# srisarya/nanopore-barcoding-ORC

Measured on AMD Instinct MI355X. Metric: Mreads/s two-round SP5×SP27 demux; % HBM roofline; 1/2/4/8 GPU, higher is better.
Workload: dtype u64

## Files before the change

### nanopore-barcoding-orc_amd/csrc/dmx_api.cpp

```cpp
#include <hip/hip_runtime.h>

#include <algorithm>
#include <atomic>
#include <cstdlib>
#include <cstdio>
#include <cstring>
#include <map>
#include <mutex>
#include <thread>
#include <tuple>
#include <utility>
#include <vector>

#include "dmx_internal.h"
#include "pack.h"

using namespace dmx;

#define CK(call)                                                                        \
    do {                                                                                \
        hipError_t e_ = (call);                                                         \
        if (e_ != hipSuccess) {                                                         \
            c->err = std::string(#call) + ": " + hipGetErrorString(e_);                 \
            return DMX_E_HIP;                                                           \
// ... 38 lines not shown


size_t counts_size(const Ctx* c) {
    const size_t a1 = c->mode == DMX_MODE_SINGLE ? 0 : (size_t)c->panel[1].n;
    return ((size_t)c->panel[0].n + 1) * (a1 + 1) + 2;
}

int ensure_pipeline(Ctx* c) {
    const size_t n = c->n_reads;
    const bool linked = c->mode == DMX_MODE_LINKED;
    const size_t slots0 = linked ? n * (size_t)std::max(1, c->panel[0].n) : n;
    const size_t items = linked ? slots0 : n;
    const size_t need = std::max(slots0, items) * (linked ? 1 : 2);
    if (!c->d_res || c->res_cap < n) {
        int rc;
        if ((rc = dev_alloc(c, &c->d_res, n))) return rc;
        c->res_cap = n;
    }
    if (c->slot_cap < need || c->cap_reads < n) {
        const size_t s = need;
        int rc;
        for (int r = 0; r < 2; ++r) {
            if ((rc = dev_alloc(c, &c->d_winner[r], s))) return rc;
            if ((rc = dev_alloc(c, &c->d_origin[r], s))) return rc;
            if ((rc = dev_alloc(c, &c->d_lb[r], s))) return rc;
        }
        if ((rc = dev_alloc(c, &c->d_linked, n))) return rc;
        c->slot_cap = s;
        c->cap_reads = n;
    }
    if (c->item_alloc < items) {
        int rc;
        if ((rc = dev_alloc(c, &c->d_items, items))) return rc;
        c->item_alloc = items;
    }
    c->item_cap = items;
    const size_t want_cl = 4 * std::max(slots0, n) + 65536;
    if (c->cl_cap < want_cl) {
        int rc;
        for (int r = 0; r < 2; ++r) {
            if ((rc = dev_alloc(c, &c->d_cl[r], want_cl))) return rc;
            if ((rc = dev_alloc(c, &c->d_outc[r], want_cl))) return rc;
        }
        c->cl_cap = want_cl;
    }
    const size_t want_cand = 4 * std::max(slots0, n) + 65536;
    if (c->cand_cap < want_cand) {
        int rc;
        for (int r = 0; r < 2; ++r)
            for (int l = 0; l < 2; ++l) {
                if ((rc = dev_alloc(c, &c->d_cand[r][l], want_cand))) return rc;
                if ((rc = dev_alloc(c, &c->d_cand_out[r][l], want_cand))) return rc;
            }
        c->cand_cap = want_cand;
    }
    const size_t want_win = 4 * 2 * std::max(slots0, n) + 65536;
    if (c->win_cap < want_win) {
        int rc;
        if ((rc = dev_alloc(c, &c->d_win, want_win))) return rc;
        if ((rc = dev_alloc(c, &c->d_win2, want_win))) return rc;
        if ((rc = dev_alloc(c, &c->d_tasks, 4 * want_win))) return rc;
        if ((rc = dev_alloc(c, &c->d_ftask, want_win))) return rc;
        c->win_cap = want_win;
        c->task_cap = 4 * want_win;
        c->ftask_cap = want_win;
    }
    const size_t want_stage = std::min<size_t>(c->win_cap, 2 * std::max(slots0, n) + 65536);
    if (c->use_stage && c->stage_cap < want_stage) {
        int rc;
        if ((rc = dev_alloc(c, &c->d_stage, want_stage * kStageWords))) return rc;
        c->stage_cap = want_stage;
    }
    const size_t nc = counts_size(c);
    if (c->n_counts != nc) {
        int rc;
// ... 16 lines not shown
                                          : x >= kShTasks ? c->task_cap : c->win_cap) /
                                         kShards);
        uint64_t t = 0;
        for (int s = 0; s < kShards; ++s) {
            const uint32_t v = sh[(size_t)(x * kShards + s) * kShardStride];
            t += std::min(v, scap);
            if (v > scap) o |= cand ? 8 : 4;
        }
        const int slot = x < kShWin2 ? 4 + x : x < kShTasks ? 10 + (x - kShWin2)
                       : x < kShCand ? 12 + (x - kShTasks) : x < kShFtask ? 6 + (x - kShCand)
                       : 14 + (x - kShFtask);
        cnt[slot] = (uint32_t)t;
    }
    if (ovf) *ovf = o;
    return hipSuccess;
}

int grow_cands(Ctx* c) {
    const size_t want = c->cand_cap * 2;
    int rc;
    for (int r = 0; r < 2; ++r)
        for (int l = 0; l < 2; ++l) {
            if ((rc = dev_alloc(c, &c->d_cand[r][l], want))) return rc;
            if ((rc = dev_alloc(c, &c->d_cand_out[r][l], want))) return rc;
        }
    c->cand_cap = want;
    return DMX_OK;
}

int grow_windows(Ctx* c) {
    const size_t want = c->win_cap * 2;
    int rc;
    if ((rc = dev_alloc(c, &c->d_win, want))) return rc;
    if ((rc = dev_alloc(c, &c->d_win2, want))) return rc;
    if ((rc = dev_alloc(c, &c->d_tasks, 4 * want))) return rc;
    if ((rc = dev_alloc(c, &c->d_ftask, want))) return rc;
    c->win_cap = want;
    c->task_cap = 4 * want;
    c->ftask_cap = want;
    return DMX_OK;
}

int grow_clusters(Ctx* c) {
    const size_t want = c->cl_cap * 2;
    int rc;
    for (int r = 0; r < 2; ++r) {
        if ((rc = dev_alloc(c, &c->d_cl[r], want))) return rc;
// ... 98 lines not shown
    hipMalloc((void**)&c->d_shard, kShLists * kShards * kShardStride * sizeof(uint32_t));
    *out = c;
    return DMX_OK;
}

void dmx_close(dmx_ctx* c) {
    if (!c) return;
    hipSetDevice(c->device);
    hipStreamSynchronize(c->stream);
    chop_release(c);
    pd_release(c);
    comm_release(c);
    void* bufs[] = {c->d_seq_alloc, c->d_nmask_alloc,     c->d_offs,     c->d_lens,      c->d_res,
                    c->d_winner[0], c->d_winner[1], c->d_origin[0], c->d_origin[1], c->d_lb[0], c->d_lb[1], c->d_cl[0],
                    c->d_cl[1],     c->d_outc[0],   c->d_outc[1],  c->d_items, c->d_win, c->d_win2, c->d_linked, c->d_tasks, c->d_counters, c->d_shard,
                    c->d_counts,    c->d_panel[0],  c->d_panel[1], c->d_pieces[0], c->d_pieces[1],
                    c->d_ftask, c->d_stage, c->d_pieces_flat, c->d_cells[0], c->d_cells[1], c->d_cells[2],
                    c->d_cells[3]};
    for (void* b : bufs)
        if (b) hipFree(b);
    for (int r = 0; r < 2; ++r)
        for (int l = 0; l < 2; ++l) {
            if (c->d_cand[r][l]) hipFree(c->d_cand[r][l]);
            if (c->d_cand_out[r][l]) hipFree(c->d_cand_out[r][l]);
        }
    void* alt[] = {c->alt.seq_alloc, c->alt.nmask_alloc, c->alt.offs, c->alt.lens, c->alt.res,
                   c->alt.exc, c->d_exc};
    for (void* b : alt)
        if (b) hipFree(b);
    for (auto& e : c->ev)
        if (e) hipEventDestroy(e);
    if (c->cstream) hipStreamDestroy(c->cstream);
    if (c->dstream) hipStreamDestroy(c->dstream);
    hipStreamDestroy(c->stream);
    delete c;
}

const char* dmx_last_error(dmx_ctx* c) {
    if (c) return c->err.c_str();
    thread_local std::string msg;
    msg = dmx::process_error();
    if (msg.empty()) msg = "null context";
    return msg.c_str();
}

int dmx_set_mode(dmx_ctx* c, int mode) {
    if (!c) return DMX_E_INVALID;
// ... 1194 lines not shown
```

### nanopore-barcoding-orc_amd/csrc/dmx_device.h

```cpp
#pragma once
#include <hip/hip_runtime.h>
#include <stdint.h>

namespace dmx {

constexpr int kMaxAdapters = 64;
constexpr int kMaxLen = 64;
constexpr int kRingSmall = 74;
constexpr int kRingLarge = 128;
constexpr int kScanBlock = 256;
constexpr int kResolveBlock = 64;

enum : uint8_t { kFront = 1, kBack = 2 };

struct DevAdapter {
    uint64_t peq[8];
    int8_t acc[72];
    int8_t pacc[72];
    uint8_t m;
    uint8_t k;
    uint8_t where;
    int8_t kk;
    uint8_t pad[4];
};
// ... 154 lines not shown
    uint32_t n, start, len;
    uint8_t strand, o, a, clean;
    uint64_t off;
};
static_assert(sizeof(Cand) == 40 && offsetof(Cand, off) == 32, "Cand layout");

struct Outcome {
    uint64_t key;
    int32_t origin;
    int32_t pad;
};

__host__ __device__ inline uint64_t make_key(int score, int o, int cost, int a, uint64_t t) {
    const int s = score < -128 ? -128 : score;
    return ((uint64_t)(127 - s) << 56) | ((uint64_t)o << 55) | ((uint64_t)cost << 48) |
           ((uint64_t)a << 40) | (t & ((1ull << 40) - 1));
}
__host__ __device__ inline int key_score(uint64_t k) { return 127 - (int)(k >> 56); }
__host__ __device__ inline int key_orient(uint64_t k) { return (int)((k >> 55) & 1); }
__host__ __device__ inline int key_cost(uint64_t k) { return (int)((k >> 48) & 127); }
__host__ __device__ inline int key_adapter(uint64_t k) { return (int)((k >> 40) & 255); }
__host__ __device__ inline uint64_t key_t(uint64_t k) { return k & ((1ull << 40) - 1); }

enum BoundsBuf : uint32_t {
    kBufSeq = 1, kBufMask = 2, kBufSlot = 3, kBufItem = 4, kBufRes = 5, kBufCount = 6,
    kBufRead = 7, kBufLinked = 8, kBufCand = 9, kBufChop = 10, kBufPd = 11,
    kBufPaTrace = 12, kBufPaOps = 13, kBufGaCols = 14, kBufRdCols = 15
};
enum BoundsKernel : int32_t {
    kKerFilter = 1, kKerVerify, kKerScreen, kKerScreen4, kKerWscan, kKerScan, kKerBand0,
    kKerBand1, kKerSelectCand, kKerResolve, kKerSelect, kKerFin0, kKerFin1, kKerFin0L, kKerFin1L,
    kKerFin2L, kKerChop, kKerChopBig, kKerChopStart, kKerSelfTest, kKerPieces, kKerPairdist,
    kKerPairalign, kKerPairalignTb, kKerGroupalign, kKerGroupalignTb, kKerGroupalignMerge,
    kKerRowdist
};
constexpr int kBoundsRec = 24;

struct Bounds {
#ifdef DMX_DEBUG_BOUNDS
    int64_t lo, hi;
    uint64_t slots, items, reads, counts, linked;
    uint32_t* rec;
    int32_t kid;
#endif
};

__device__ __forceinline__ bool bchk(const Bounds& b, int64_t i, int64_t lo, int64_t hi,
                                     uint32_t buf) {
#ifdef DMX_DEBUG_BOUNDS
    if (i >= lo && i < hi) return true;
    atomicOr(b.rec + 3, 32u);
    if (atomicCAS(b.rec + kBoundsRec, 0u, (uint32_t)b.kid + 1u) == 0u) {
        b.rec[kBoundsRec + 1] = buf;
        b.rec[kBoundsRec + 2] = (uint32_t)(uint64_t)i;
// ... 139 lines not shown
```

### nanopore-barcoding-orc_amd/csrc/dmx_internal.h

```cpp
#pragma once
#include <hip/hip_runtime.h>

#include <string>
#include <vector>

#include "../../include/dmx.h"
#include "dmx_device.h"

struct ncclComm;

namespace dmx {

struct ChopState;
struct PdState;
struct PaState;
struct GaState;
struct RdState;

struct PanelReach {
    int pre_raw = 0;
    int pre = 0;
    int post = 0;
    int need_pre = 0;
    int need_post = 0;
// ... 39 lines not shown
    uint32_t* d_seq_alloc = nullptr;
    uint32_t* d_nmask_alloc = nullptr;
    uint64_t* d_offs = nullptr;
    uint32_t* d_lens = nullptr;
    uint32_t* d_exc = nullptr;
    size_t exc_cap = 0;

    struct InSet {
        uint32_t* seq_alloc = nullptr;
        uint32_t* nmask_alloc = nullptr;
        uint64_t* offs = nullptr;
        uint32_t* lens = nullptr;
        dmx_result* res = nullptr;
        uint32_t* exc = nullptr;
        size_t cap_words = 0, cap_reads = 0, res_cap = 0, n_words = 0, exc_cap = 0;
    } alt;
    hipStream_t cstream = nullptr;
    hipStream_t dstream = nullptr;
    bool chunked = false;

    dmx_result* d_res = nullptr;
    unsigned long long* d_winner[2] = {nullptr, nullptr};
    int32_t* d_origin[2] = {nullptr, nullptr};
    int32_t* d_lb[2] = {nullptr, nullptr};
    bool ring_small[2] = {true, true};
    bool band_ok[2] = {true, true};
    bool band_wide[2] = {true, true};
    bool orient_slot[2] = {false, false};
    bool force_ring = false;
    size_t slot_cap = 0;
    Cluster* d_cl[2] = {nullptr, nullptr};
    Outcome* d_outc[2] = {nullptr, nullptr};
    size_t cl_cap = 0;
    Cand* d_cand[2][2] = {{nullptr, nullptr}, {nullptr, nullptr}};
    Outcome* d_cand_out[2][2] = {{nullptr, nullptr}, {nullptr, nullptr}};
    size_t cand_cap = 0;
    Window* d_win = nullptr;
    Window* d_win2 = nullptr;
    size_t win_cap = 0;
    ItemView* d_items = nullptr;
    size_t item_cap = 0;
    size_t item_alloc = 0;
    uint32_t* d_shard = nullptr;
    uint32_t* d_counters = nullptr;
    unsigned long long* d_counts = nullptr;
    unsigned long long* d_linked = nullptr;
    Window* d_tasks = nullptr;
    size_t task_cap = 0;
    uint32_t* d_stage = nullptr;
    size_t stage_cap = 0;
    bool use_stage = false;
    FTask* d_ftask = nullptr;
    size_t ftask_cap = 0;
    DevPieces* d_pieces_flat = nullptr;
    int flat_rounds = 0;
    int flat_want = 0;
    int flat_step = 0;
    size_t flat_lds = 0;
// ... 6 lines not shown
    bool screen_v1 = false;
    size_t n_counts = 0;
    hipEvent_t ev[17] = {};
    bool executed = false;
    ChopState* chop = nullptr;
    PdState* pd = nullptr;
    PaState* pa = nullptr;
    GaState* ga = nullptr;
    RdState* rd = nullptr;

    ncclComm* comm = nullptr;
    int comm_ranks = 0, comm_rank = 0;
    uint64_t comm_group = 0;
    bool counts_reduced = false;
};

void chop_release(Ctx* c);
void pd_release(Ctx* c);
void comm_release(Ctx* c);
int reset_counts(Ctx* c);
void set_process_error(const std::string& msg);
std::string process_error();
void chop_invalidate(Ctx* c);
int launch_round(Ctx* c, int round, hipStream_t st);
int prepare_flat(Ctx* c, hipStream_t st);
int launch_finalize(Ctx* c, int round, hipStream_t st);
int launch_rebase_offsets(uint64_t* offs, uint32_t n, uint64_t g0, hipStream_t st);
int launch_mask_scatter(uint32_t* mask, const uint32_t* d_exc, uint32_t n, uint32_t base,
                        hipStream_t st);

Bounds make_bounds(const Ctx* c, int kid);
inline void set_kid(Bounds& b, int kid) {
#ifdef DMX_DEBUG_BOUNDS
    b.kid = kid;
#else
    (void)b, (void)kid;
#endif
}
hipError_t bounds_reset(Ctx* c, hipStream_t st);
int bounds_check(Ctx* c, const char* where);

PanelReach panel_reach(const HostPanel& hp, const DevPanel& dp);
int bounds_selftest(Ctx* c, uint32_t* host_out);

struct MaskSrc {
    const uint32_t* dense = nullptr;
// ... 13 lines not shown
```

### nanopore-barcoding-orc_amd/csrc/dmx_kernels.hip

```cpp
#include <algorithm>
#include <cstring>
#include <memory>
#include <type_traits>
#include <utility>
#include <vector>

#include "dmx_device.h"
#include "dmx_internal.h"

namespace dmx {

struct RoundArgs {
    Packed pk;
    const uint64_t* offs;
    const uint32_t* lens;
    const DevPanel* panel;
    const ItemView* items;
    const uint32_t* n_items_dev;
    uint32_t n_items;
    int32_t T;
    int32_t per_task_slot;
    int32_t slot_div;
    Cluster* cl;
    Outcome* outc;
    uint32_t* cl_count;
    uint32_t cl_cap;
    uint32_t* flags;
    unsigned long long* winner;
    int32_t* origin;
    int32_t* lb;
    Window* win;
    uint32_t* win_count;
    uint32_t win_cap;
    uint32_t win_scap;
    Window* win2;
    uint32_t* win2_count;
    uint32_t* diag;
    int32_t band;
    Cand* cand[2];
    Outcome* cand_out[2];
    uint32_t* cand_count;
    uint32_t cand_cap;
    uint32_t cand_scap;
    int32_t screen;
    Window* tasks;
    uint32_t* task_count;
    uint32_t task_cap;
    uint32_t task_scap;
    const DevPieces* pieces;
    FTask* ftask;
    uint32_t* ftask_count;
    uint32_t ftask_scap;
    uint32_t* stage;
    uint32_t stage_cap;
    uint32_t n_words;
    uint32_t nsb;
    int32_t round;
    uint32_t* cells[4];
};

#ifndef DMX_MASK_SKIP
#define DMX_MASK_SKIP 1
#endif
// ... 3341 lines not shown
    for (int x = threadIdx.x; x < 72 * A; x += blockDim.x) s_bacc[x] = P->ad[x / 72].acc[x % 72];
    __shared__ uint32_t s_multi;
    if (threadIdx.x == 0) s_multi = 0;
    __syncthreads();
    for (int x = threadIdx.x; x < 64 * A; x += blockDim.x) {
        const int a = x >> 6, i = x & 63;
        const DevAdapter& ad = P->ad[a];
        uint32_t r = 0;
        for (int c = 0; c < 4; ++c) r |= (uint32_t)((ad.peq[c] >> i) & 1ull) << c;
        if (__popc(r) == 1) r |= (uint32_t)(__ffs(r) - 1) << 4;
        else if (i < (int)ad.m) s_multi = 1u;
        s_rm[i * kMaxAdapters + a] = (uint8_t)r;
    }
    if (threadIdx.x == 0) {
        s_nq[0] = 0;
        s_nq[1] = 0;
        s_n = 0;
    }
    __shared__ uint32_t s_spre[kShards + 1];
    ShardMap sm{s_spre, 0u};
    sm.load(R.cand_count + list * kShards * kShardStride, R.cand_scap);
    const uint32_t total = sm.total();
    const Cand* cl = R.cand[list];
    Outcome* outs = R.cand_out[list];
    const uint32_t wave = threadIdx.x >> 6;
    const bool fast = s_multi == 0;

    auto dp_pass = [&](int e, uint32_t cnt) {
        const uint32_t lo = s_nq[e] - cnt;
        if (threadIdx.x < 8) s_hist[threadIdx.x] = 0;
        __syncthreads();
        uint32_t ci = 0, cost = 0, pos = 0;
        const bool have = threadIdx.x < cnt;
        if (have) {
            ci = s_q[e][lo + threadIdx.x];
            cost = s_qc[e][lo + threadIdx.x];
            pos = atomicAdd(&s_hist[cost], 1u);
        }
        __syncthreads();
        if (have) {
            uint32_t before = 0;
            for (uint32_t c = 0; c < cost; ++c) before += s_hist[c];
            s_sorted[before + pos] = ci;
            s_sc[before + pos] = (uint8_t)cost;
        }
        __syncthreads();
        if (threadIdx.x == 0) {
// ... 18 lines not shown
                tv.n = c.n;
                tv.strand = c.strand;
                tv.clean = c.clean != 0;
                tv.start = c.start;
                tv.len = c.len;
                view_off(R.pk, c.off, tv);
                tv.o = c.o;
                tv.a = c.a;
                int c2, origin, score;
#ifdef DMX_BAND_SKIP_DP
                c2 = cst;
                origin = (int)(c.j) - iend;
                score = (int)wc;
                if (false)
#endif
                if (e == 0)
                    band_dp_cost<CMIN == 0 ? 1 : CMIN, CMAX, false>(
                        wc, fast, s_rm + c.a, R.pk, tv, ad.front, iend, j, c2,
                        origin, score);
                else
                    band_dp_cost<CMIN == 0 ? 1 : CMIN, CMAX, true>(
                        wc, fast, s_rm + c.a, R.pk, tv, ad.front, iend, j, c2,
                        origin, score);
                if (c2 != cst) atomicOr(R.flags, 2u);
                const int lr = iend + (origin < 0 ? origin : 0);
                if (slot_in && lr >= 0 && cst <= (int)acc[lr]) {
                    Outcome out;
                    out.key = make_key(score, c.o, cst, c.a, t);
                    out.origin = origin;
                    out.pad = (int32_t)slot;
                    atomicMin(&R.winner[slot], (unsigned long long)out.key);
                    outs[cj] = out;
                }
            }
        }
        __syncthreads();
    };

    for (uint32_t base = blockIdx.x * blockDim.x; base < total; base += gridDim.x * blockDim.x) {
        const uint32_t ti = base + threadIdx.x;
        const uint32_t ci = ti < total ? sm.phys(ti) : 0u;
        Cand c{};
        if (ti < total) c = cl[ci];
        if (ti < total && (cmask == 0 || ((cmask >> c.cost) & 1))) {
            const uint32_t slot = slot_of(R, c.item, c.sub);
            const bool slot_in = DMX_BOUND(R.pk.bd, slots, slot, kBufSlot);
            const int cost = c.cost, iend = c.iend;
            const int j = (int)c.j;
            const uint64_t t = iend == (int)(s_amk[c.a] & 255u) ? (uint64_t)j
                                                               : (uint64_t)c.len + 1 + iend;
            Outcome out;
            out.key = ~0ull;
            out.origin = 0;
            out.pad = 0;
            const int lrmax = min(iend, j + cost);
            const int ub = lrmax - 2 * cost;
            if (slot_in && viable_lb(R.lb[slot], lrmax, c.o, cost) &&
                make_key(ub, c.o, cost, c.a, t) <= R.winner[slot]) {
                if (cost == 0) {
                    const int origin = j - iend;
                    const int score = j >= iend ? iend : j;
                    const int lr = iend + (origin < 0 ? origin : 0);
                    if (lr >= 0 && 0 <= (int)s_bacc[72 * c.a + lr]) {
                        out.key = make_key(score, c.o, 0, c.a, t);
                        out.origin = origin;
                        out.pad = (int32_t)slot;
                        atomicMin(&R.winner[slot], (unsigned long long)out.key);
                    }
                } else {
                    const int dx = j - iend;
                    const int H = CMAX;
                    const int e = (dx - H < 0 || j + H > (int)c.len) ? 1 : 0;
                    const uint32_t q = atomicAdd(&s_nq[e], 1u);
                    s_q[e][q] = ci;
                    s_qc[e][q] = (uint8_t)cost;
                }
            }
            outs[ci] = out;
        }
        __syncthreads();
        for (int e = 0; e < 2; ++e)
            while (s_nq[e] >= 256u) dp_pass(e, 256u);
        __syncthreads();
    }
    for (int e = 0; e < 2; ++e)
        if (s_nq[e]) dp_pass(e, s_nq[e]);
    if (threadIdx.x == 0 && s_n) atomicAdd(R.diag + 1, s_n);
}

__global__ void select_cand_kernel(RoundArgs R) {
    __shared__ uint32_t s_spre[kShards + 1];
    for (int list = 0; list < 2; ++list) {
        ShardMap sm{s_spre, 0u};
        __syncthreads();
        sm.load(R.cand_count + list * kShards * kShardStride, R.cand_scap);
        const uint32_t total = sm.total();
        for (uint32_t ti = blockIdx.x * blockDim.x + threadIdx.x; ti < total;
             ti += gridDim.x * blockDim.x) {
            const uint32_t ci = sm.phys(ti);
            const Outcome o = R.cand_out[list][ci];
            if (o.key == ~0ull) continue;
            const uint32_t slot = (uint32_t)o.pad;
            if (!DMX_BOUND(R.pk.bd, slots, slot, kBufSlot)) continue;
            if (R.winner[slot] == o.key) R.origin[slot] = o.origin;
        }
    }
}

__global__ void select_kernel(RoundArgs R) {
    const uint32_t total = min(*R.cl_count, R.cl_cap);
    for (uint32_t ci = blockIdx.x * blockDim.x + threadIdx.x; ci < total;
         ci += gridDim.x * blockDim.x) {
        const Outcome o = R.outc[ci];
        if (o.key == ~0ull) continue;
        const Cluster c = R.cl[ci];
        const uint32_t slot = slot_of(R, c.item, c.sub);
        if (!DMX_BOUND(R.pk.bd, slots, slot, kBufSlot)) continue;
        if (R.winner[slot] == o.key) R.origin[slot] = o.origin;
    }
}

__device__ __forceinline__ void decode_match(uint64_t key, int origin, uint32_t vlen,
                                             const DevPanel* P, dmx_match& mt, int& a, int& o) {
    a = key_adapter(key);
    o = key_orient(key);
    const uint64_t t = key_t(key);
    int refstop, qstop;
    if (t <= vlen) {
        qstop = (int)t;
        refstop = P->ad[a].m;
    } else {
        refstop = (int)(t - vlen - 1);
        qstop = (int)vlen;
    }
    mt.rstop = qstop;
    mt.astop = (int16_t)refstop;
    if (origin >= 0) {
        mt.astart = 0;
        mt.rstart = origin;
    } else {
        mt.astart = (int16_t)(-origin);
        mt.rstart = 0;
    }
    mt.score = (int16_t)key_score(key);
    mt.errors = (int16_t)key_cost(key);
}

struct FinalArgs {
    const uint32_t* lens;
    const DevPanel* p0;
    const DevPanel* p1;
    const unsigned long long* winner;
    const int32_t* origin;
    dmx_result* res;
    ItemView* items;
    uint32_t* n_items;
    uint32_t n_reads;
    int32_t mode;
    int32_t A0, A1;
    int32_t oslot;
    unsigned long long* counts;
    const unsigned long long* winner0;
    const int32_t* origin0;
    unsigned long long* linked_best;
    Bounds bd;
};

__global__ __launch_bounds__(256) void finalize0_linked_kernel(FinalArgs F) {
    __shared__ uint32_t s_nq, s_qbase;
    if (threadIdx.x == 0) s_nq = 0;
    __syncthreads();
    const uint32_t r = blockIdx.x * blockDim.x + threadIdx.x;
    uint32_t nmine = 0, qi = 0;
    uint32_t n = 0;
    if (r < F.n_reads && DMX_BOUND(F.bd, reads, r, kBufRes) &&
        DMX_BOUND(F.bd, linked, r, kBufLinked) &&
        DMX_BOUND(F.bd, slots, (size_t)r * F.A0 + F.A0 - 1, kBufSlot)) {
        dmx_result out;
        out.bin1 = out.bin2 = -1;
        out.rc1 = out.rc2 = 0;
        out.flags = 0;
        out._pad = 0;
        out.m1 = dmx_match{0, 0, 0, 0, 0, 0};
        out.m2 = out.m1;
        F.res[r] = out;
        F.linked_best[r] = ~0ull;
        n = F.lens[r];
        for (int a = 0; a < F.A0; ++a) nmine += F.winner[(size_t)r * F.A0 + a] != ~0ull;
        if (nmine) qi = atomicAdd(&s_nq, nmine);
    }
    __syncthreads();
    if (threadIdx.x == 0) s_qbase = s_nq ? atomicAdd(F.n_items, s_nq) : 0u;
    __syncthreads();
    if (nmine) {
        uint32_t idx = s_qbase + qi;
        for (int a = 0; a < F.A0; ++a) {
            const uint64_t key = F.winner[(size_t)r * F.A0 + a];
            if (key == ~0ull) continue;
            dmx_match m;
            int aa, o;
            decode_match(key, F.origin[(size_t)r * F.A0 + a], n, F.p0, m, aa, o);
            ItemView v;
            v.read = r;
            v.strand = 0;
            v.pad = 0;
            v.only_adapter = (int16_t)a;
            v.start = (uint32_t)m.rstop;
            v.len = n - (uint32_t)m.rstop;
            if (DMX_BOUND(F.bd, items, idx, kBufItem)) F.items[idx] = v;
            ++idx;
        }
    }
}

__global__ __launch_bounds__(256) void finalize1_linked_kernel(FinalArgs F) {
    const uint32_t i = blockIdx.x * blockDim.x + threadIdx.x;
    if (i >= *F.n_items) return;
    if (!DMX_BOUND(F.bd, items, i, kBufItem) || !DMX_BOUND(F.bd, slots, i, kBufSlot)) return;
    const ItemView v = F.items[i];
    const uint64_t kb = F.winner[i];
    if (kb == ~0ull) return;
    const int a = v.only_adapter;
    if (!DMX_BOUND(F.bd, linked, v.read, kBufLinked)) return;
    const uint64_t kf = F.winner0[(size_t)v.read * F.A0 + a];
// ... 1 lines not shown
    const int err = key_cost(kf) + key_cost(kb);
    const uint64_t ck = ((uint64_t)(511 - sum) << 54) | ((uint64_t)err << 46) |
                        ((uint64_t)a << 38) | (uint64_t)i;
    atomicMin(&F.linked_best[v.read], (unsigned long long)ck);
}

__global__ __launch_bounds__(256) void finalize2_linked_kernel(FinalArgs F) {
    __shared__ unsigned int s_hist[kMaxAdapters + 1];
    for (int x = threadIdx.x; x <= F.A0; x += blockDim.x) s_hist[x] = 0;
    __syncthreads();
    for (uint32_t r = blockIdx.x * blockDim.x + threadIdx.x; r < F.n_reads;
         r += gridDim.x * blockDim.x) {
        const uint64_t ck = DMX_BOUND(F.bd, linked, r, kBufLinked) ? F.linked_best[r] : ~0ull;
        int b = -1;
        if (ck != ~0ull) {
            const uint32_t i = (uint32_t)(ck & ((1ull << 38) - 1));
            const int a = (int)((ck >> 38) & 255);
            if (!DMX_BOUND(F.bd, items, i, kBufItem) || !DMX_BOUND(F.bd, slots, i, kBufSlot) ||
                !DMX_BOUND(F.bd, reads, r, kBufRes))
                continue;
            const ItemView v = F.items[i];
            dmx_result& out = F.res[r];
            int aa, o;
            decode_match(F.winner0[(size_t)r * F.A0 + a], F.origin0[(size_t)r * F.A0 + a],
                         F.lens[r], F.p0, out.m1, aa, o);
            decode_match(F.winner[i], F.origin[i], v.len, F.p1, out.m2, aa, o);
            out.bin1 = out.bin2 = (int16_t)a;
            b = a;
        }
        atomicAdd(&s_hist[b + 1], 1u);
    }
    __syncthreads();
    for (int x = threadIdx.x; x <= F.A0; x += blockDim.x)
        if (s_hist[x] && DMX_BOUND(F.bd, counts, x * (F.A0 + 1) + x, kBufCount))
            atomicAdd(&F.counts[x * (F.A0 + 1) + x], (unsigned long long)s_hist[x]);
}

__device__ __forceinline__ uint32_t pick_winner(const FinalArgs& F, uint32_t i, uint64_t& key,
                                                int& o) {
    if (!DMX_BOUND(F.bd, slots, F.oslot ? 2 * (uint64_t)i + 1 : i, kBufSlot)) {
        key = ~0ull;
        o = 0;
        return 0;
    }
    if (!F.oslot) {
        key = F.winner[i];
        o = key != ~0ull ? key_orient(key) : 0;
        return i;
    }
// ... 16 lines not shown
    if (threadIdx.x == 0) s_nq = 0;
    __syncthreads();
    uint32_t n_rc = 0;
    for (uint32_t base = blockIdx.x * 256u; base < F.n_reads; base += gridDim.x * 256u) {
        const uint32_t r = base + threadIdx.x;
        ItemView v;
        uint32_t qi = ~0u;
        if (r < F.n_reads && DMX_BOUND(F.bd, reads, r, kBufRes)) {
            dmx_result out;
            out.bin1 = -1;
            out.bin2 = -1;
            out.rc1 = out.rc2 = 0;
            out.flags = 0;
            out._pad = 0;
            out.m1 = dmx_match{0, 0, 0, 0, 0, 0};
            out.m2 = out.m1;
            uint64_t key;
            int o;
            const uint32_t ws = pick_winner(F, r, key, o);
            out.rc1 = (uint8_t)o;
            if (key != ~0ull) {
                int a;
                const uint32_t n = F.lens[r];
                decode_match(key, F.origin[ws], n, F.p0, out.m1, a, o);
                out.bin1 = (int16_t)a;
                out.rc1 = (uint8_t)o;
                if (F.mode == DMX_MODE_TWO_ROUND) {
                    v.read = r;
                    v.strand = (uint8_t)o;
                    v.pad = 0;
                    v.only_adapter = -1;
                    if (F.p0->ad[a].where == kFront) {
                        v.start = (uint32_t)out.m1.rstop;
                        v.len = n - (uint32_t)out.m1.rstop;
                    } else {
                        v.start = 0;
                        v.len = (uint32_t)out.m1.rstart;
                    }
                    qi = atomicAdd(&s_nq, 1u);
                } else {
                    atomicAdd(&s_hist[a + 1], 1u);
                }
            } else {
                atomicAdd(&s_hist[0], 1u);
            }
            n_rc += o ? 1u : 0u;
            F.res[r] = out;
// ... 19 lines not shown
            atomicAdd(&F.counts[ix], (unsigned long long)v);
    }
}

__global__ __launch_bounds__(256) void finalize1_kernel(FinalArgs F) {
    extern __shared__ unsigned int s_hist2[];
    const int nbins = (F.A0 + 1) * (F.A1 + 1);
    for (int x = threadIdx.x; x < nbins + 1; x += blockDim.x) s_hist2[x] = 0;
    __syncthreads();
    const uint32_t n_items = *F.n_items;
    uint32_t n_rc = 0;
    for (uint32_t i = blockIdx.x * 256u + threadIdx.x; i < n_items; i += gridDim.x * 256u) {
        if (!DMX_BOUND(F.bd, items, i, kBufItem)) break;
        const ItemView v = F.items[i];
        if (!DMX_BOUND(F.bd, reads, v.read, kBufRes)) continue;
        dmx_result& out = F.res[v.read];
        uint64_t key;
        int o;
        const uint32_t ws = pick_winner(F, i, key, o);
        int b = -1;
        out.rc2 = (uint8_t)o;
        if (key != ~0ull) {
            int a;
            decode_match(key, F.origin[ws], v.len, F.p1, out.m2, a, o);
            out.bin2 = (int16_t)a;
            b = a;
        }
        n_rc += o ? 1u : 0u;
        atomicAdd(&s_hist2[(out.bin1 + 1) * (F.A1 + 1) + (b + 1)], 1u);
    }
    n_rc = wave_sum(n_rc);
    if ((threadIdx.x & 63u) == 0 && n_rc) atomicAdd(&s_hist2[nbins], n_rc);
    __syncthreads();
    for (int x = threadIdx.x; x < nbins + 1; x += blockDim.x) {
        const unsigned int c = s_hist2[x];
        const int ix = x == nbins ? nbins + 1 : x;
        if (c && DMX_BOUND(F.bd, counts, ix, kBufCount))
            atomicAdd(&F.counts[ix], (unsigned long long)c);
    }
}

static int resolve_grid(const Ctx* c) {
    (void)c;
    return 256 * 8;
}

static bool debug_sync() {
// ... 24 lines not shown
    b.linked = c->cap_reads;
    b.rec = c->d_counters;
    b.kid = kid;
#else
    (void)c, (void)kid;
#endif
    return b;
}

hipError_t bounds_reset(Ctx* c, hipStream_t st) {
#ifdef DMX_DEBUG_BOUNDS
    return hipMemsetAsync(c->d_counters + kBoundsRec, 0, 4 * sizeof(uint32_t), st);
#else
    (void)c, (void)st;
    return hipSuccess;
#endif
}

int bounds_check(Ctx* c, const char* where) {
#ifdef DMX_DEBUG_BOUNDS
    static const char* const kKer[] = {
        "?", "filter_kernel", "verify_kernel", "iscreen_kernel", "iscreen4_kernel",
        "wscan_kernel", "scan_kernel", "band_cand_kernel<0,3>", "band_cand_kernel<4,5|7>",
        "select_cand_kernel", "resolve_kernel", "select_kernel", "finalize0_kernel",
        "finalize1_kernel", "finalize0_linked_kernel", "finalize1_linked_kernel",
        "finalize2_linked_kernel", "chop_kernel", "chop_big_kernel", "chop_start",
        "bounds_selftest_kernel", "pscreen_kernel", "pairdist_kernel", "pairalign_kernel",
        "pairalign_traceback_kernel", "groupalign_kernel", "groupalign_traceback_kernel",
        "groupalign_merge_kernel", "rowdist_kernel"};
    static const char* const kBuf[] = {"?", "seq", "nmask", "winner slots", "items", "results",
                                       "counts", "reads", "linked keys", "candidates", "chop",
                                       "pairdist scratch", "pairalign trace", "pairalign ops",
                                       "groupalign columns", "rowdist columns"};
    uint32_t rec[4];
    hipError_t e = hipStreamSynchronize(c->stream);
    if (e == hipSuccess)
        e = hipMemcpy(rec, c->d_counters + kBoundsRec, sizeof(rec), hipMemcpyDeviceToHost);
    if (e != hipSuccess) {
        c->err = std::string(where) + ": " + hipGetErrorString(e);
        return DMX_E_HIP;
    }
    if (!rec[0]) return DMX_OK;
    const int k = (int)rec[0] - 1;
    const int64_t idx = (int64_t)(((uint64_t)rec[3] << 32) | rec[2]);
    char msg[256];
    snprintf(msg, sizeof msg, "%s: bounds violation in %s: %s index %lld outside its buffer",
             where, k > 0 && k < (int)(sizeof kKer / sizeof *kKer) ? kKer[k] : "?",
             rec[1] < sizeof kBuf / sizeof *kBuf ? kBuf[rec[1]] : "?", (long long)idx);
// ... 145 lines not shown
    }
    R.cl = c->d_cl[round];
    R.outc = c->d_outc[round];
    R.cl_count = c->d_counters + round;
    R.cl_cap = (uint32_t)c->cl_cap;
    R.flags = c->d_counters + 3;
    R.winner = c->d_winner[round];
    R.origin = c->d_origin[round];
    R.lb = c->d_lb[round];
    if (R.T > kScanBlock) return DMX_E_UNSUPPORTED;
    hipMemsetAsync(R.lb, 0, sizeof(int32_t) * (round == 0 ? c->slot_cap
                                                         : c->item_cap * (R.slot_div ? 2 : 1)),
                   st);

    const uint32_t rpb = kScanBlock / R.T;
    const uint32_t grid = (uint32_t)((R.n_items + rpb - 1) / rpb);
    R.diag = c->d_counters + 16 + 4 * round;
    R.win = c->d_win;
    R.win_count = c->d_shard + (kShWin + round) * kShards * kShardStride;
    R.win2 = c->d_win2;
    R.win2_count = c->d_shard + (kShWin2 + round) * kShards * kShardStride;
    R.win_cap = (uint32_t)c->win_cap;
    R.win_scap = (uint32_t)(c->win_cap / kShards);
    const bool band = c->band_ok[round] && !c->force_ring;
    R.band = band ? 1 : 0;
    for (int l = 0; l < 2; ++l) {
        R.cand[l] = c->d_cand[round][l];
        R.cand_out[l] = c->d_cand_out[round][l];
    }
    R.cand_count = c->d_shard + (kShCand + 2 * round) * kShards * kShardStride;
    R.cand_cap = (uint32_t)c->cand_cap;
    R.cand_scap = (uint32_t)(c->cand_cap / kShards);
    R.screen = (hp.filter && hp.verify && hp.screen && !linked && !c->no_screen &&
                (uint64_t)c->win_cap * (uint64_t)hp.n < (1ull << 32)) ? 1 : 0;
    R.tasks = c->d_tasks;
    R.task_count = c->d_shard + (kShTasks + round) * kShards * kShardStride;
    R.task_cap = (uint32_t)c->task_cap;
    R.task_scap = (uint32_t)(c->task_cap / kShards);
    R.pieces = c->d_pieces[round];
    R.ftask = c->d_ftask;
    R.ftask_count = c->d_shard + (kShFtask + round) * kShards * kShardStride;
    R.ftask_scap = (uint32_t)(c->ftask_cap / kShards);
    R.stage = (DMX_STAGE_SLOTS && c->d_stage && !linked && hp.filter && band && c->use_stage &&
               (uint64_t)c->n_words * 16 < (1ull << kOffBits))
                  ? c->d_stage : nullptr;
    R.stage_cap = (uint32_t)c->stage_cap;
    R.pk.stage = c->d_stage;
    R.n_words = (uint32_t)c->n_words;
    R.nsb = (uint32_t)((c->n_words + kSuperNt / 16 - 1) / (kSuperNt / 16));
    R.round = round;
    for (int i = 0; i < 4; ++i)
// ... 92 lines not shown
        if (band) hipLaunchKernelGGL(scan_kernel<true>, dim3(grid), dim3(kScanBlock), 0, st, R);
        else hipLaunchKernelGGL(scan_kernel<false>, dim3(grid), dim3(kScanBlock), 0, st, R);
        DMX_DBG_SYNC("scan_kernel");
    }
    hipEventRecord(c->ev[round * 3 + 1], st);
    if (band) {
        set_kid(R.pk.bd, kKerBand0);
        hipLaunchKernelGGL((band_cand_kernel<0, 3>), dim3(256 * 8), dim3(256), 0, st, R, 0, 0);
        DMX_DBG_SYNC("band_cand_kernel<0, 3>");
        set_kid(R.pk.bd, kKerBand1);
        if (c->band_wide[round] && kBandSplit) {
            hipLaunchKernelGGL((band_cand_kernel<4, 7>), dim3(256 * 4), dim3(256), 0, st, R, 1, 16);
            hipLaunchKernelGGL((band_cand_kernel<4, 7>), dim3(256 * 4), dim3(256), 0, st, R, 1, 32);
            hipLaunchKernelGGL((band_cand_kernel<4, 7>), dim3(256 * 4), dim3(256), 0, st, R, 1, 192);
        } else if (c->band_wide[round]) {
            hipLaunchKernelGGL((band_cand_kernel<4, 7>), dim3(256 * 4), dim3(256), 0, st, R, 1, 0);
        } else if (kBandSplit) {
            hipLaunchKernelGGL((band_cand_kernel<4, 5>), dim3(256 * 4), dim3(256), 0, st, R, 1, 16);
            hipLaunchKernelGGL((band_cand_kernel<4, 5>), dim3(256 * 4), dim3(256), 0, st, R, 1, 32);
        } else {
            hipLaunchKernelGGL((band_cand_kernel<4, 5>), dim3(256 * 4), dim3(256), 0, st, R, 1, 0);
        }
        DMX_DBG_SYNC("band_cand_kernel<4, 5|7>");
        set_kid(R.pk.bd, kKerSelectCand);
        hipLaunchKernelGGL(select_cand_kernel, dim3(1024), dim3(256), 0, st, R);
        DMX_DBG_SYNC("select_cand_kernel");
        hipEventRecord(c->ev[round * 3 + 2], st);
        return hipGetLastError() == hipSuccess ? DMX_OK : DMX_E_HIP;
    }
    const size_t tabs = (size_t)144 * hp.n;
    static bool attr_set = false;
    if (!attr_set) {
        hipFuncSetAttribute((const void*)resolve_kernel<kRingSmall>,
                            hipFuncAttributeMaxDynamicSharedMemorySize, 160 * 1024);
        hipFuncSetAttribute((const void*)resolve_kernel<kRingLarge>,
                            hipFuncAttributeMaxDynamicSharedMemorySize, 160 * 1024);
        attr_set = true;
    }
    set_kid(R.pk.bd, kKerResolve);
    if (c->ring_small[round])
        hipLaunchKernelGGL(resolve_kernel<kRingSmall>, dim3(resolve_grid(c)), dim3(kResolveBlock),
                           (size_t)kRingSmall * kResolveBlock * 16 + tabs, st, R);
    else
        hipLaunchKernelGGL(resolve_kernel<kRingLarge>, dim3(resolve_grid(c)), dim3(kResolveBlock),
                           (size_t)kRingLarge * kResolveBlock * 16 + tabs, st, R);
    DMX_DBG_SYNC("resolve_kernel");
    set_kid(R.pk.bd, kKerSelect);
    hipLaunchKernelGGL(select_kernel, dim3(1024), dim3(256), 0, st, R);
    DMX_DBG_SYNC("select_kernel");
// ... 14 lines not shown

int launch_rebase_offsets(uint64_t* offs, uint32_t n, uint64_t g0, hipStream_t st) {
    if (!n) return DMX_OK;
    const uint32_t grid = min((n + 255u) / 256u, 2048u);
    hipLaunchKernelGGL(rebase_offsets_kernel, dim3(grid), dim3(256), 0, st, offs, n, g0);
    return hipGetLastError() == hipSuccess ? DMX_OK : DMX_E_HIP;
}

int launch_mask_scatter(uint32_t* mask, const uint32_t* d_exc, uint32_t n, uint32_t base,
                        hipStream_t st) {
    if (!n) return DMX_OK;
    const uint32_t grid = min((n + 255u) / 256u, 1024u);
    hipLaunchKernelGGL(mask_scatter_kernel, dim3(grid), dim3(256), 0, st, mask, d_exc, n, base);
    return hipGetLastError() == hipSuccess ? DMX_OK : DMX_E_HIP;
}

int launch_finalize(Ctx* c, int round, hipStream_t st) {
    FinalArgs F;
    F.lens = c->d_lens;
    F.p0 = c->d_panel[0];
    F.p1 = c->d_panel[1];
    F.winner = c->d_winner[round];
    F.origin = c->d_origin[round];
    F.res = c->d_res;
    F.items = c->d_items;
    F.n_items = c->d_counters + 2;
    F.n_reads = (uint32_t)c->n_reads;
    F.mode = c->mode;
    F.A0 = c->panel[0].n;
    F.A1 = c->mode == DMX_MODE_SINGLE ? 0 : c->panel[1].n;
    F.oslot = c->orient_slot[round] ? 1 : 0;
    F.counts = c->d_counts;
    F.winner0 = c->d_winner[0];
    F.origin0 = c->d_origin[0];
    F.linked_best = c->d_linked;
    F.bd = make_bounds(c, kKerFin0);
    if (c->mode == DMX_MODE_LINKED) {
        const uint32_t gr = (uint32_t)((c->n_reads + 255) / 256);
        if (round == 0) {
            set_kid(F.bd, kKerFin0L);
            if (gr) hipLaunchKernelGGL(finalize0_linked_kernel, dim3(gr), dim3(256), 0, st, F);
        } else {
            const uint32_t gi = (uint32_t)((c->item_cap + 255) / 256);
            set_kid(F.bd, kKerFin1L);
            if (gi) hipLaunchKernelGGL(finalize1_linked_kernel, dim3(gi), dim3(256), 0, st, F);
            set_kid(F.bd, kKerFin2L);
            if (gr)
                hipLaunchKernelGGL(finalize2_linked_kernel, dim3(std::min(gr, kFinalGrid)),
                                   dim3(256), 0, st, F);
        }
        DMX_DBG_SYNC("finalize_linked");
        hipEventRecord(c->ev[6 + round], st);
        return hipGetLastError() == hipSuccess ? DMX_OK : DMX_E_HIP;
    }
    if (round == 0) {
        const uint32_t grid = (uint32_t)std::min<size_t>((c->n_reads + 255) / 256, kFinalGrid);
        if (grid) hipLaunchKernelGGL(finalize0_kernel, dim3(grid), dim3(256), 0, st, F);
// ... 13 lines not shown
```

Before: 339.2.

## Pack alignment origin delta into winner key, drop select_cand pass

Encodes the alignment origin as a small biased delta in the low bits of the 64-bit winner key, so the atomicMin winner alone carries the origin. This removes the per-candidate Outcome array writes, the select_cand_kernel launch, and the origin buffers on the band path, cutting memory traffic and one kernel per round. Finalize decodes the origin from the key when the band path ran. Cases whose delta or cost does not fit the code now set the fallback flag, and the ring path keeps using the separate origin buffer.

```diff
diff --git a/nanopore-barcoding-orc_amd/csrc/dmx_api.cpp b/nanopore-barcoding-orc_amd/csrc/dmx_api.cpp
--- a/nanopore-barcoding-orc_amd/csrc/dmx_api.cpp
+++ b/nanopore-barcoding-orc_amd/csrc/dmx_api.cpp
@@ -84,12 +84,20 @@
         int rc;
         for (int r = 0; r < 2; ++r) {
             if ((rc = dev_alloc(c, &c->d_winner[r], s))) return rc;
-            if ((rc = dev_alloc(c, &c->d_origin[r], s))) return rc;
             if ((rc = dev_alloc(c, &c->d_lb[r], s))) return rc;
         }
         if ((rc = dev_alloc(c, &c->d_linked, n))) return rc;
         c->slot_cap = s;
         c->cap_reads = n;
+    }
+    for (int r = 0; r < 2; ++r) {
+        if ((r == 1 && c->mode == DMX_MODE_SINGLE) || band_round(c, r) ||
+            c->origin_cap[r] >= c->slot_cap)
+            continue;
+        c->origin_cap[r] = 0;
+        int rc;
+        if ((rc = dev_alloc(c, &c->d_origin[r], c->slot_cap))) return rc;
+        c->origin_cap[r] = c->slot_cap;
     }
     if (c->item_alloc < items) {
         int rc;
@@ -112,7 +120,6 @@
         for (int r = 0; r < 2; ++r)
             for (int l = 0; l < 2; ++l) {
                 if ((rc = dev_alloc(c, &c->d_cand[r][l], want_cand))) return rc;
-                if ((rc = dev_alloc(c, &c->d_cand_out[r][l], want_cand))) return rc;
             }
         c->cand_cap = want_cand;
     }
@@ -175,7 +182,6 @@
     for (int r = 0; r < 2; ++r)
         for (int l = 0; l < 2; ++l) {
             if ((rc = dev_alloc(c, &c->d_cand[r][l], want))) return rc;
-            if ((rc = dev_alloc(c, &c->d_cand_out[r][l], want))) return rc;
         }
     c->cand_cap = want;
     return DMX_OK;
@@ -320,7 +326,6 @@
     for (int r = 0; r < 2; ++r)
         for (int l = 0; l < 2; ++l) {
             if (c->d_cand[r][l]) hipFree(c->d_cand[r][l]);
-            if (c->d_cand_out[r][l]) hipFree(c->d_cand_out[r][l]);
         }
     void* alt[] = {c->alt.seq_alloc, c->alt.nmask_alloc, c->alt.offs, c->alt.lens, c->alt.res,
                    c->alt.exc, c->d_exc};
diff --git a/nanopore-barcoding-orc_amd/csrc/dmx_device.h b/nanopore-barcoding-orc_amd/csrc/dmx_device.h
--- a/nanopore-barcoding-orc_amd/csrc/dmx_device.h
+++ b/nanopore-barcoding-orc_amd/csrc/dmx_device.h
@@ -200,6 +200,26 @@
 __host__ __device__ inline int key_adapter(uint64_t k) { return (int)((k >> 40) & 255); }
 __host__ __device__ inline uint64_t key_t(uint64_t k) { return k & ((1ull << 40) - 1); }
 
+constexpr int kKeyPosBits = 40;
+constexpr int kKeyDeltaBits = 4;
+constexpr int kKeyDeltaBias = 8;
+constexpr int kKeyDeltaMin = -kKeyDeltaBias;
+constexpr int kBandMaxCost = 7;
+static_assert(sizeof(uint32_t) * 8 + 1 <= kKeyPosBits - kKeyDeltaBits,
+              "t = len + 1 + iend < 2^33 must fit above the delta code");
+static_assert(kBandMaxCost < kKeyDeltaBias && kBandMaxCost + kKeyDeltaBias < (1 << kKeyDeltaBits),
+              "|delta| <= cost <= 7 must fit the delta code");
+__host__ __device__ inline uint64_t make_key_o(int score, int o, int cost, int a, uint64_t t,
+                                               int delta) {
+    return make_key(score, o, cost, a,
+                    (t << kKeyDeltaBits) |
+                        (uint64_t)((delta + kKeyDeltaBias) & ((1 << kKeyDeltaBits) - 1)));
+}
+__host__ __device__ inline uint64_t key_t_o(uint64_t k) { return key_t(k) >> kKeyDeltaBits; }
+__host__ __device__ inline int key_delta(uint64_t k) {
+    return (int)(k & ((1u << kKeyDeltaBits) - 1)) - kKeyDeltaBias;
+}
+
 enum BoundsBuf : uint32_t {
     kBufSeq = 1, kBufMask = 2, kBufSlot = 3, kBufItem = 4, kBufRes = 5, kBufCount = 6,
     kBufRead = 7, kBufLinked = 8, kBufCand = 9, kBufChop = 10, kBufPd = 11,
@@ -207,7 +227,7 @@
 };
 enum BoundsKernel : int32_t {
     kKerFilter = 1, kKerVerify, kKerScreen, kKerScreen4, kKerWscan, kKerScan, kKerBand0,
-    kKerBand1, kKerSelectCand, kKerResolve, kKerSelect, kKerFin0, kKerFin1, kKerFin0L, kKerFin1L,
+    kKerBand1, kKerResolve, kKerSelect, kKerFin0, kKerFin1, kKerFin0L, kKerFin1L,
     kKerFin2L, kKerChop, kKerChopBig, kKerChopStart, kKerSelfTest, kKerPieces, kKerPairdist,
     kKerPairalign, kKerPairalignTb, kKerGroupalign, kKerGroupalignTb, kKerGroupalignMerge,
     kKerRowdist
diff --git a/nanopore-barcoding-orc_amd/csrc/dmx_internal.h b/nanopore-barcoding-orc_amd/csrc/dmx_internal.h
--- a/nanopore-barcoding-orc_amd/csrc/dmx_internal.h
+++ b/nanopore-barcoding-orc_amd/csrc/dmx_internal.h
@@ -85,6 +85,7 @@
     dmx_result* d_res = nullptr;
     unsigned long long* d_winner[2] = {nullptr, nullptr};
     int32_t* d_origin[2] = {nullptr, nullptr};
+    size_t origin_cap[2] = {0, 0};
     int32_t* d_lb[2] = {nullptr, nullptr};
     bool ring_small[2] = {true, true};
     bool band_ok[2] = {true, true};
@@ -96,7 +97,6 @@
     Outcome* d_outc[2] = {nullptr, nullptr};
     size_t cl_cap = 0;
     Cand* d_cand[2][2] = {{nullptr, nullptr}, {nullptr, nullptr}};
-    Outcome* d_cand_out[2][2] = {{nullptr, nullptr}, {nullptr, nullptr}};
     size_t cand_cap = 0;
     Window* d_win = nullptr;
     Window* d_win2 = nullptr;
@@ -149,6 +149,7 @@
 void set_process_error(const std::string& msg);
 std::string process_error();
 void chop_invalidate(Ctx* c);
+inline bool band_round(const Ctx* c, int round) { return c->band_ok[round] && !c->force_ring; }
 int launch_round(Ctx* c, int round, hipStream_t st);
 int prepare_flat(Ctx* c, hipStream_t st);
 int launch_finalize(Ctx* c, int round, hipStream_t st);
diff --git a/nanopore-barcoding-orc_amd/csrc/dmx_kernels.hip b/nanopore-barcoding-orc_amd/csrc/dmx_kernels.hip
--- a/nanopore-barcoding-orc_amd/csrc/dmx_kernels.hip
+++ b/nanopore-barcoding-orc_amd/csrc/dmx_kernels.hip
@@ -38,7 +38,6 @@
     uint32_t* diag;
     int32_t band;
     Cand* cand[2];
-    Outcome* cand_out[2];
     uint32_t* cand_count;
     uint32_t cand_cap;
     uint32_t cand_scap;
@@ -3426,7 +3425,6 @@
     sm.load(R.cand_count + list * kShards * kShardStride, R.cand_scap);
     const uint32_t total = sm.total();
     const Cand* cl = R.cand[list];
-    Outcome* outs = R.cand_out[list];
     const uint32_t wave = threadIdx.x >> 6;
     const bool fast = s_multi == 0;
 
@@ -3491,16 +3489,12 @@
                     band_dp_cost<CMIN == 0 ? 1 : CMIN, CMAX, true>(
                         wc, fast, s_rm + c.a, R.pk, tv, ad.front, iend, j, c2,
                         origin, score);
-                if (c2 != cst) atomicOr(R.flags, 2u);
+                const int delta = origin - (j - iend);
+                if (c2 != cst || abs(delta) > cst || cst > kBandMaxCost) atomicOr(R.flags, 2u);
                 const int lr = iend + (origin < 0 ? origin : 0);
-                if (slot_in && lr >= 0 && cst <= (int)acc[lr]) {
-                    Outcome out;
-                    out.key = make_key(score, c.o, cst, c.a, t);
-                    out.origin = origin;
-                    out.pad = (int32_t)slot;
-                    atomicMin(&R.winner[slot], (unsigned long long)out.key);
-                    outs[cj] = out;
-                }
+                if (slot_in && lr >= 0 && cst <= (int)acc[lr])
+                    atomicMin(&R.winner[slot],
+                              (unsigned long long)make_key_o(score, c.o, cst, c.a, t, delta));
             }
         }
         __syncthreads();
@@ -3518,24 +3512,17 @@
             const int j = (int)c.j;
             const uint64_t t = iend == (int)(s_amk[c.a] & 255u) ? (uint64_t)j
                                                                : (uint64_t)c.len + 1 + iend;
-            Outcome out;
-            out.key = ~0ull;
-            out.origin = 0;
-            out.pad = 0;
             const int lrmax = min(iend, j + cost);
             const int ub = lrmax - 2 * cost;
             if (slot_in && viable_lb(R.lb[slot], lrmax, c.o, cost) &&
-                make_key(ub, c.o, cost, c.a, t) <= R.winner[slot]) {
+                make_key_o(ub, c.o, cost, c.a, t, kKeyDeltaMin) <= R.winner[slot]) {
                 if (cost == 0) {
                     const int origin = j - iend;
                     const int score = j >= iend ? iend : j;
                     const int lr = iend + (origin < 0 ? origin : 0);
-                    if (lr >= 0 && 0 <= (int)s_bacc[72 * c.a + lr]) {
-                        out.key = make_key(score, c.o, 0, c.a, t);
-                        out.origin = origin;
-                        out.pad = (int32_t)slot;
-                        atomicMin(&R.winner[slot], (unsigned long long)out.key);
-                    }
+                    if (lr >= 0 && 0 <= (int)s_bacc[72 * c.a + lr])
+                        atomicMin(&R.winner[slot],
+                                  (unsigned long long)make_key_o(score, c.o, 0, c.a, t, 0));
                 } else {
                     const int dx = j - iend;
                     const int H = CMAX;
@@ -3545,7 +3532,6 @@
                     s_qc[e][q] = (uint8_t)cost;
                 }
             }
-            outs[ci] = out;
         }
         __syncthreads();
         for (int e = 0; e < 2; ++e)
@@ -3555,25 +3541,6 @@
     for (int e = 0; e < 2; ++e)
         if (s_nq[e]) dp_pass(e, s_nq[e]);
     if (threadIdx.x == 0 && s_n) atomicAdd(R.diag + 1, s_n);
-}
-
-__global__ void select_cand_kernel(RoundArgs R) {
-    __shared__ uint32_t s_spre[kShards + 1];
-    for (int list = 0; list < 2; ++list) {
-        ShardMap sm{s_spre, 0u};
-        __syncthreads();
-        sm.load(R.cand_count + list * kShards * kShardStride, R.cand_scap);
-        const uint32_t total = sm.total();
-        for (uint32_t ti = blockIdx.x * blockDim.x + threadIdx.x; ti < total;
-             ti += gridDim.x * blockDim.x) {
-            const uint32_t ci = sm.phys(ti);
-            const Outcome o = R.cand_out[list][ci];
-            if (o.key == ~0ull) continue;
-            const uint32_t slot = (uint32_t)o.pad;
-            if (!DMX_BOUND(R.pk.bd, slots, slot, kBufSlot)) continue;
-            if (R.winner[slot] == o.key) R.origin[slot] = o.origin;
-        }
-    }
 }
 
 __global__ void select_kernel(RoundArgs R) {
@@ -3589,11 +3556,12 @@
     }
 }
 
-__device__ __forceinline__ void decode_match(uint64_t key, int origin, uint32_t vlen,
-                                             const DevPanel* P, dmx_match& mt, int& a, int& o) {
+__device__ __forceinline__ void decode_match(uint64_t key, bool okey, const int32_t* origins,
+                                             size_t slot, uint32_t vlen, const DevPanel* P,
+                                             dmx_match& mt, int& a, int& o) {
     a = key_adapter(key);
     o = key_orient(key);
-    const uint64_t t = key_t(key);
+    const uint64_t t = okey ? key_t_o(key) : key_t(key);
     int refstop, qstop;
     if (t <= vlen) {
         qstop = (int)t;
@@ -3604,6 +3572,7 @@
     }
     mt.rstop = qstop;
     mt.astop = (int16_t)refstop;
+    const int origin = okey ? qstop - refstop + key_delta(key) : origins[slot];
     if (origin >= 0) {
         mt.astart = 0;
         mt.rstart = origin;
@@ -3621,6 +3590,7 @@
     const DevPanel* p1;
     const unsigned long long* winner;
     const int32_t* origin;
+    int32_t okey;
     dmx_result* res;
     ItemView* items;
     uint32_t* n_items;
@@ -3631,6 +3601,7 @@
     unsigned long long* counts;
     const unsigned long long* winner0;
     const int32_t* origin0;
+    int32_t okey0;
     unsigned long long* linked_best;
     Bounds bd;
 };
@@ -3668,7 +3639,7 @@
             if (key == ~0ull) continue;
             dmx_match m;
             int aa, o;
-            decode_match(key, F.origin[(size_t)r * F.A0 + a], n, F.p0, m, aa, o);
+            decode_match(key, F.okey, F.origin, (size_t)r * F.A0 + a, n, F.p0, m, aa, o);
             ItemView v;
             v.read = r;
             v.strand = 0;
@@ -3716,9 +3687,9 @@
             const ItemView v = F.items[i];
             dmx_result& out = F.res[r];
             int aa, o;
-            decode_match(F.winner0[(size_t)r * F.A0 + a], F.origin0[(size_t)r * F.A0 + a],
-                         F.lens[r], F.p0, out.m1, aa, o);
-            decode_match(F.winner[i], F.origin[i], v.len, F.p1, out.m2, aa, o);
+            decode_match(F.winner0[(size_t)r * F.A0 + a], F.okey0, F.origin0,
+                         (size_t)r * F.A0 + a, F.lens[r], F.p0, out.m1, aa, o);
+            decode_match(F.winner[i], F.okey, F.origin, i, v.len, F.p1, out.m2, aa, o);
             out.bin1 = out.bin2 = (int16_t)a;
             b = a;
         }
@@ -3781,7 +3752,7 @@
             if (key != ~0ull) {
                 int a;
                 const uint32_t n = F.lens[r];
-                decode_match(key, F.origin[ws], n, F.p0, out.m1, a, o);
+                decode_match(key, F.okey, F.origin, ws, n, F.p0, out.m1, a, o);
                 out.bin1 = (int16_t)a;
                 out.rc1 = (uint8_t)o;
                 if (F.mode == DMX_MODE_TWO_ROUND) {
@@ -3847,7 +3818,7 @@
         out.rc2 = (uint8_t)o;
         if (key != ~0ull) {
             int a;
-            decode_match(key, F.origin[ws], v.len, F.p1, out.m2, a, o);
+            decode_match(key, F.okey, F.origin, ws, v.len, F.p1, out.m2, a, o);
             out.bin2 = (int16_t)a;
             b = a;
         }
@@ -3918,8 +3889,7 @@
     static const char* const kKer[] = {
         "?", "filter_kernel", "verify_kernel", "iscreen_kernel", "iscreen4_kernel",
         "wscan_kernel", "scan_kernel", "band_cand_kernel<0,3>", "band_cand_kernel<4,5|7>",
-        "select_cand_kernel", "resolve_kernel", "select_kernel", "finalize0_kernel",
-        "finalize1_kernel", "finalize0_linked_kernel", "finalize1_linked_kernel",
+        "resolve_kernel", "select_kernel", "finalize0_kernel", "finalize1_kernel", "finalize0_linked_kernel", "finalize1_linked_kernel",
         "finalize2_linked_kernel", "chop_kernel", "chop_big_kernel", "chop_start",
         "bounds_selftest_kernel", "pscreen_kernel", "pairdist_kernel", "pairalign_kernel",
         "pairalign_traceback_kernel", "groupalign_kernel", "groupalign_traceback_kernel",
@@ -4111,11 +4081,10 @@
     R.win2_count = c->d_shard + (kShWin2 + round) * kShards * kShardStride;
     R.win_cap = (uint32_t)c->win_cap;
     R.win_scap = (uint32_t)(c->win_cap / kShards);
-    const bool band = c->band_ok[round] && !c->force_ring;
+    const bool band = band_round(c, round);
     R.band = band ? 1 : 0;
     for (int l = 0; l < 2; ++l) {
         R.cand[l] = c->d_cand[round][l];
-        R.cand_out[l] = c->d_cand_out[round][l];
     }
     R.cand_count = c->d_shard + (kShCand + 2 * round) * kShards * kShardStride;
     R.cand_cap = (uint32_t)c->cand_cap;
@@ -4254,9 +4223,6 @@
             hipLaunchKernelGGL((band_cand_kernel<4, 5>), dim3(256 * 4), dim3(256), 0, st, R, 1, 0);
         }
         DMX_DBG_SYNC("band_cand_kernel<4, 5|7>");
-        set_kid(R.pk.bd, kKerSelectCand);
-        hipLaunchKernelGGL(select_cand_kernel, dim3(1024), dim3(256), 0, st, R);
-        DMX_DBG_SYNC("select_cand_kernel");
         hipEventRecord(c->ev[round * 3 + 2], st);
         return hipGetLastError() == hipSuccess ? DMX_OK : DMX_E_HIP;
     }
@@ -4317,6 +4283,7 @@
     F.p1 = c->d_panel[1];
     F.winner = c->d_winner[round];
     F.origin = c->d_origin[round];
+    F.okey = band_round(c, round) ? 1 : 0;
     F.res = c->d_res;
     F.items = c->d_items;
     F.n_items = c->d_counters + 2;
@@ -4328,6 +4295,7 @@
     F.counts = c->d_counts;
     F.winner0 = c->d_winner[0];
     F.origin0 = c->d_origin[0];
+    F.okey0 = band_round(c, 0) ? 1 : 0;
     F.linked_best = c->d_linked;
     F.bd = make_bounds(c, kKerFin0);
     if (c->mode == DMX_MODE_LINKED) {
```

After: 346.4, median of 6. 1.02x the previous value.
